# rust-control/oxide_control

Hardware: NVIDIA B200
Metric: env-steps/sec (higher is better)
Workload: dtype f32

## Files before the change

oxide_control_b200/csrc/ox_jit.cpp:

```cpp
#include <cuda_runtime_api.h>
#include <sys/stat.h>
#include <unistd.h>

#include <atomic>
#include <cerrno>
#include <cinttypes>
#include <cstdio>
#include <cstdlib>
#include <fstream>
#include <map>
#include <memory>
#include <mutex>
#include <sstream>
#include <string>
#include <vector>

#include "ox_specsrc.h"

#define OX_INCBIN(sym, file)                                                                                       \
  __asm__(".section .rodata\n.hidden " #sym "\n.global " #sym "\n.balign 16\n" #sym ":\n.incbin \"" file "\"\n"   \
          ".hidden " #sym "_end\n.global " #sym "_end\n" #sym "_end:\n.byte 0\n.previous\n");                      \
  extern "C" const char sym[];                                                                                     \
  extern "C" const char sym##_end[];
OX_INCBIN(ox_embed_spec_cuh, "ox_spec.cuh")
OX_INCBIN(ox_embed_stages_cuh, "ox_stages.cuh")
OX_INCBIN(ox_embed_blob_h, "ox_blob.h")
OX_INCBIN(ox_embed_abi_h, "../../include/ox_b200.h")

namespace ox {
namespace {

const char* kFlags = "-std=c++17 -O3 -lineinfo -gencode arch=compute_100a,code=sm_100a --expt-relaxed-constexpr -cubin";

struct Embedded { const char* rel; const char* begin; const char* end; };
const Embedded* embedded(int* n) {
  static const Embedded e[] = {
      {"src/csrc/ox_spec.cuh", ox_embed_spec_cuh, ox_embed_spec_cuh_end},
      {"src/csrc/ox_stages.cuh", ox_embed_stages_cuh, ox_embed_stages_cuh_end},
      {"src/csrc/ox_blob.h", ox_embed_blob_h, ox_embed_blob_h_end},
      {"include/ox_b200.h", ox_embed_abi_h, ox_embed_abi_h_end},
  };
  *n = 4;
  return e;
}

uint64_t fnv(uint64_t h, const void* p, size_t n) {
  const unsigned char* c = static_cast<const unsigned char*>(p);
  for (size_t i = 0; i < n; i++) { h ^= c[i]; h *= 1099511628211ull; }
  return h;
}
uint64_t abi_hash() {
  static const uint64_t h = [] {
    uint64_t x = 1469598103934665603ull;
    int n;
    const Embedded* e = embedded(&n);
    for (int i = 0; i < n; i++) x = fnv(x, e[i].begin, (size_t)(e[i].end - e[i].begin));
    x = fnv(x, kFlags, strlen(kFlags));
    return x;
  }();
  return h;
}

bool mkdirs(const std::string& path) {
  std::string cur;
  for (size_t i = 0; i <= path.size(); i++) {
    if (i == path.size() || path[i] == '/') {
      if (!cur.empty() && mkdir(cur.c_str(), 0755) != 0 && errno != EEXIST) return false;
    }
    if (i < path.size()) cur += path[i];
  }
  return true;
}
bool write_file(const std::string& path, const char* data, size_t n) {
  std::ofstream f(path, std::ios::binary);
  if (!f) return false;
  f.write(data, (std::streamsize)n);
  return (bool)f;
}
bool read_file(const std::string& path, std::vector<char>* out) {
  std::ifstream f(path, std::ios::binary);
  if (!f) return false;
  out->assign(std::istreambuf_iterator<char>(f), std::istreambuf_iterator<char>());
  return !out->empty();
}
std::string cache_dir() {
  if (const char* d = getenv("OX_B200_CACHE_DIR")) if (*d) return d;
  if (const char* d = getenv("XDG_CACHE_HOME")) if (*d) return std::string(d) + "/ox_b200";
  if (const char* d = getenv("HOME")) if (*d) return std::string(d) + "/.cache/ox_b200";
  return "/tmp/ox_b200_cache";
}
std::string find_nvcc() {
  auto ok = [](const std::string& p) { return !p.empty() && access(p.c_str(), X_OK) == 0; };
  if (const char* p = getenv("OX_B200_NVCC")) if (ok(p)) return p;
  for (const char* v : {"CUDA_HOME", "CUDA_PATH"})
    if (const char* d = getenv(v)) { std::string p = std::string(d) + "/bin/nvcc"; if (ok(p)) return p; }
  if (ok("/usr/local/cuda/bin/nvcc")) return "/usr/local/cuda/bin/nvcc";
  if (const char* path = getenv("PATH")) {
    std::stringstream ss(path);
    std::string dir;
    while (std::getline(ss, dir, ':')) { std::string p = dir + "/nvcc"; if (ok(p)) return p; }
  }
  return "";
}
std::string shq(const std::string& s) {
  std::string r = "'";
  for (char c : s) { if (c == '\'') r += "'\\''"; else r += c; }
  return r + "'";
}
std::string tail(const std::string& path, size_t n) {
  std::vector<char> d;
  if (!read_file(path, &d)) return "";
  return std::string(d.size() > n ? d.end() - (long)n : d.begin(), d.end());
}

bool compile_unit(const ox_model_tables& t, bool f64, const std::string& cubin, std::string* why) {
  const std::string nvcc = find_nvcc();
  if (nvcc.empty()) { *why = "nvcc not found (set OX_B200_NVCC or CUDA_HOME)"; return false; }
  static std::atomic<int> counter{0};
  const std::string dir = cache_dir();
  char tmpname[64];
  snprintf(tmpname, sizeof tmpname, "/build_%ld_%d", (long)getpid(), counter++);
  const std::string work = dir + tmpname;
  if (!mkdirs(work + "/src/csrc") || !mkdirs(work + "/include")) { *why = "cannot create " + work; return false; }
  int n;
  const Embedded* e = embedded(&n);
  for (int i = 0; i < n; i++)
    if (!write_file(work + "/" + e[i].rel, e[i].begin, (size_t)(e[i].end - e[i].begin))) { *why = "cannot write " + work + "/" + e[i].rel; return false; }
  const std::string src = spec_source_jit(t, f64);
  if (!write_file(work + "/src/csrc/spec.cu", src.data(), src.size())) { *why = "cannot write spec.cu"; return false; }
  const std::string cmd = shq(nvcc) + " " + kFlags + " -I" + shq(work + "/src/csrc") + " -o " + shq(work + "/spec.cubin") + " " +
                          shq(work + "/src/csrc/spec.cu") + " > " + shq(work + "/nvcc.log") + " 2>&1";
  const int rc = system(cmd.c_str());
  std::vector<char> probe;
  if (rc != 0 || !read_file(work + "/spec.cubin", &probe)) {
    *why = "nvcc failed (rc " + std::to_string(rc) + "): " + tail(work + "/nvcc.log", 600) + " [sources kept in " + work + "]";
    return false;
  }
  if (rename((work + "/spec.cubin").c_str(), cubin.c_str()) != 0) { *why = "cannot move the cubin into " + cubin; return false; }
  const std::string rm = "rm -rf " + shq(work);
  if (system(rm.c_str()) != 0) {  }
  return true;
}

struct JitEntry {
  SpecEntry spec;
  std::string name;
  cudaLibrary_t lib[2] = {nullptr, nullptr};
  std::string cubin[2];
};
std::mutex g_mu;
std::map<uint64_t, std::unique_ptr<JitEntry>>& table() {
  static std::map<uint64_t, std::unique_ptr<JitEntry>> t;
  return t;
}

}

bool jit_enabled() {
  const char* v = getenv("OX_B200_JIT");
  return !(v && v[0] == '0');
}

const SpecEntry* jit_spec(const ox_model_tables& t, bool f64, bool allow_compile, bool load, std::string* why, std::string* cubin_path) {
  std::string dummy;
  if (!why) why = &dummy;
  if (!jit_enabled()) { *why = "run-time specialisation disabled (OX_B200_JIT=0)"; return nullptr; }
  const uint64_t hash = model_hash(t);
  std::lock_guard<std::mutex> lock(g_mu);
  auto& slot = table()[hash];
  if (!slot) {
    slot.reset(new JitEntry);
    char nm[64];
    snprintf(nm, sizeof nm, "jit_%016" PRIx64, hash);
    slot->name = nm;
    slot->spec.hash = hash;
    slot->spec.name = slot->name.c_str();
  }
  JitEntry& je = *slot;
  const int p = f64 ? 1 : 0;
  void** kern = f64 ? je.spec.jit_f64 : je.spec.jit_f32;
  if (je.cubin[p].empty()) {
    const std::string dir = cache_dir();
    if (!mkdirs(dir)) { *why = "cannot create the cache directory " + dir; return nullptr; }
    char fn[128];
    snprintf(fn, sizeof fn, "/ox_%016" PRIx64 "_%s_%016" PRIx64 ".cubin", hash, f64 ? "f64" : "f32", abi_hash());
    const std::string path = dir + fn;
    if (access(path.c_str(), R_OK) != 0) {
      if (!allow_compile) { *why = "no cached cubin for this model (" + path + ")"; return nullptr; }
      if (!compile_unit(t, f64, path, why)) return nullptr;
    }
    je.cubin[p] = path;
  }
  if (cubin_path) *cubin_path = je.cubin[p];
  if (!load) return &je.spec;
  if (!kern[0]) {
    std::vector<char> image;
    if (!read_file(je.cubin[p], &image)) { *why = "cannot read " + je.cubin[p]; return nullptr; }
    cudaLibrary_t lib = nullptr;
    cudaError_t err = cudaLibraryLoadData(&lib, image.data(), nullptr, nullptr, 0, nullptr, nullptr, 0);
    if (err != cudaSuccess) { *why = std::string("cudaLibraryLoadData: ") + cudaGetErrorString(err); cudaGetLastError(); return nullptr; }
    cudaKernel_t k0 = nullptr, k1 = nullptr, k2 = nullptr;
    err = cudaLibraryGetKernel(&k0, lib, "ox_jit_step");
    if (err != cudaSuccess) { *why = std::string("cudaLibraryGetKernel(ox_jit_step): ") + cudaGetErrorString(err); cudaGetLastError(); cudaLibraryUnload(lib); return nullptr; }
    if (spec_wants_split(t)) {
      if (cudaLibraryGetKernel(&k1, lib, "ox_jit_pre") != cudaSuccess || cudaLibraryGetKernel(&k2, lib, "ox_jit_post") != cudaSuccess) {
        cudaGetLastError(); k1 = k2 = nullptr;
      }
    }
    je.lib[p] = lib;
// ... 8 lines not shown
```

oxide_control_b200/csrc/ox_stages.cuh:

```cuda
#pragma once
#include <cmath>

#include "ox_blob.h"

namespace ox {

OX_HD float ox_sqrt(float x) { return sqrtf(x); }
OX_HD double ox_sqrt(double x) { return sqrt(x); }
OX_HD float ox_rsqrt(float x) {
#if defined(__CUDA_ARCH__)
  return rsqrtf(x);
#else
  return 1.0f / sqrtf(x);
#endif
}
OX_HD double ox_rsqrt(double x) {
#if defined(__CUDA_ARCH__)
  return rsqrt(x);
#else
  return 1.0 / sqrt(x);
#endif
}
OX_HD float ox_abs(float x) { return fabsf(x); }
OX_HD double ox_abs(double x) { return fabs(x); }
// ... 1696 lines not shown
          if (!body) continue;
          const int last_ = m.body_dofadr(body) + m.body_dofnum(body) - 1;
          OX_MLOOP
          for (int d_ = 0, dof = last_; d_ < m.dof_depth(last_); d_++, dof = m.dof_parentid(dof)) {
            T cd[6];
            ld<6>(cd, b.cdof, 6 * dof);
            OX_MLOOP
            for (int k = 0; k < 3; k++) at(b.efc_J, (q0 + k) * nv + dof) += sign * (G[3 * k] * cd[0] + G[3 * k + 1] * cd[1] + G[3 * k + 2] * cd[2]);
          }
        }
        const T rdiag = m.body_invweight0(2 * b1 + 1) + m.body_invweight0(2 * b2 + 1);
        OX_MLOOP
        for (int k = 0; k < 3; k++) eq_row_finish(i, q0 + k, res[k], rdiag);
      }
    } else {
      const int j1 = m.eq_obj1id(i), j2 = m.eq_obj2id(i);
      const int d1 = m.jnt_dofadr(j1), q1 = m.jnt_qposadr(j1);
      const int r = nefc++;
      OX_MLOOP
      for (int k = 0; k < nv; k++) at(b.efc_J, r * nv + k) = 0;
      T c[5];
      OX_LDM(5, c, eq_data, 11 * i);
      T pos = at(b.qpos, q1) - m.qpos0(q1), diag = m.dof_invweight0(d1);
      at(b.efc_J, r * nv + d1) = 1;
      if (j2 >= 0) {
        const int d2 = m.jnt_dofadr(j2), q2 = m.jnt_qposadr(j2);
        const T dq = at(b.qpos, q2) - m.qpos0(q2);
        pos -= c[0] + dq * (c[1] + dq * (c[2] + dq * (c[3] + dq * c[4])));
        at(b.efc_J, r * nv + d2) = -(c[1] + dq * (2 * c[2] + dq * (3 * c[3] + dq * 4 * c[4])));
        diag += m.dof_invweight0(d2);
      } else {
        pos -= c[0];
      }
      eq_row_finish(i, r, pos, diag);
    }
  }
  OX_HD void friction_row(int i, int& nefc) const {
    const T fl = m.dof_frictionloss(i);
    if (!(fl > 0)) return;
    const int nv = m.h().nv, r = nefc++;
    OX_MLOOP
    for (int k = 0; k < nv; k++) at(b.efc_J, r * nv + k) = 0;
    at(b.efc_J, r * nv + i) = 1;
    T aref, sr[2], si[5];
    OX_LDM(2, sr, dof_solref_fri, 2 * i);
    OX_LDM(5, si, dof_solimp_fri, 5 * i);
    const T R = row_params(sr, si, (T)0, (T)0, m.dof_invweight0(i), at(b.qvel, i), &aref);
    at(b.efc_pos, r) = 0; at(b.efc_margin, r) = 0; at(b.efc_D, r) = 1 / R; at(b.efc_aref, r) = aref; at(b.efc_floss, r) = fl;
  }
  OX_HD T ball_angle_axis(int j, T* axis) const {
    T q[4];
    ld<4>(q, b.qpos, m.jnt_qposadr(j));
    normalize4(q);
    const T sn = ox_sqrt(q[1] * q[1] + q[2] * q[2] + q[3] * q[3]);
    T ang = 2 * ox_atan2(sn, q[0]);
    if (ang > (T)3.14159265358979323846) ang -= (T)(2 * 3.14159265358979323846);
    const T inv = sn > (T)OX_MINVAL ? 1 / sn : (T)0;
    const T sg = ang < 0 ? (T)-1 : (T)1;
    axis[0] = sg * q[1] * inv; axis[1] = sg * q[2] * inv; axis[2] = sg * q[3] * inv;
    return ox_abs(ang);
  }
  OX_HD int limit_count(int j) const {
    if (!m.jnt_limited(j)) return 0;
    const int jt = m.jnt_type(j);
    if (jt == OX_JNT_BALL) {
      T axis[3];
      return ox_max(m.jnt_range(2 * j), m.jnt_range(2 * j + 1)) - ball_angle_axis(j, axis) < m.jnt_margin(j) ? 1 : 0;
    }
    if (jt != OX_JNT_SLIDE && jt != OX_JNT_HINGE) return 0;
    const T value = at(b.qpos, m.jnt_qposadr(j)), margin = m.jnt_margin(j);
    return (value - m.jnt_range(2 * j) < margin ? 1 : 0) + (m.jnt_range(2 * j + 1) - value < margin ? 1 : 0);
  }
  OX_HD void limit_rows(int j, int& nefc) const {
    const int nv = m.h().nv;
    {
      {
          if (!m.jnt_limited(j)) return;
          const int jt = m.jnt_type(j);
          if (jt == OX_JNT_BALL) {
            T axis[3];
            const T margin = m.jnt_margin(j), dist = ox_max(m.jnt_range(2 * j), m.jnt_range(2 * j + 1)) - ball_angle_axis(j, axis);
            if (!(dist < margin)) return;
            const int da = m.jnt_dofadr(j), r = nefc++;
            OX_MLOOP
            for (int i = 0; i < nv; i++) at(b.efc_J, r * nv + i) = 0;
            T vel = 0;
            OX_MLOOP
            for (int k = 0; k < 3; k++) { at(b.efc_J, r * nv + da + k) = -axis[k]; vel -= axis[k] * at(b.qvel, da + k); }
            T aref, sr[2], si[5];
            OX_LDM(2, sr, jnt_solref, 2 * j);
            OX_LDM(5, si, jnt_solimp, 5 * j);
            const T R = row_params(sr, si, dist, margin, m.dof_invweight0(da), vel, &aref);
            at(b.efc_pos, r) = dist; at(b.efc_margin, r) = margin; at(b.efc_D, r) = 1 / R; at(b.efc_aref, r) = aref;
            return;
          }
          if (jt != OX_JNT_SLIDE && jt != OX_JNT_HINGE) return;
          const int da = m.jnt_dofadr(j);
          const T value = at(b.qpos, m.jnt_qposadr(j)), margin = m.jnt_margin(j);
          OX_MLOOP
          for (int side = -1; side <= 1; side += 2) {
            const T dist = side * (m.jnt_range(2 * j + (side + 1) / 2) - value);
            if (dist < margin) {
              const int r = nefc++;
              OX_MLOOP
              for (int i = 0; i < nv; i++) at(b.efc_J, r * nv + i) = 0;
              at(b.efc_J, r * nv + da) = (T)(-side);
              const T vel = (T)(-side) * at(b.qvel, da);
              T aref;
              T sr[2], si[5];
              OX_LDM(2, sr, jnt_solref, 2 * j);
              OX_LDM(5, si, jnt_solimp, 5 * j);
              const T R = row_params(sr, si, dist, margin, m.dof_invweight0(da), vel, &aref);
              at(b.efc_pos, r) = dist; at(b.efc_margin, r) = margin; at(b.efc_D, r) = 1 / R; at(b.efc_aref, r) = aref;
            }
          }
      }
    }
  }

  OX_HD int tendon_limit_count(int i) const {
    if (!m.tendon_limited(i)) return 0;
    const T value = at(b.ten_length, i), margin = m.tendon_margin(i);
    return (value - m.tendon_range(2 * i) < margin ? 1 : 0) + (m.tendon_range(2 * i + 1) - value < margin ? 1 : 0);
  }
  OX_HD void tendon_limit_rows(int i, int& nefc) const {
    const int nv = m.h().nv;
    if (!m.tendon_limited(i)) return;
    const T value = at(b.ten_length, i), margin = m.tendon_margin(i);
    OX_MLOOP
    for (int side = -1; side <= 1; side += 2) {
      const T dist = side * (m.tendon_range(2 * i + (side + 1) / 2) - value);
      if (dist < margin) {
        const int r = nefc++;
        OX_MLOOP
        for (int k = 0; k < nv; k++) at(b.efc_J, r * nv + k) = 0;
        T vel = 0;
        OX_MLOOP
        for (int k = 0; k < nv; k++) {
          const T c = (T)(-side) * at(b.ten_J, i * nv + k);
          at(b.efc_J, r * nv + k) = c;
          vel += c * at(b.qvel, k);
        }
        T aref, sr[2], si[5];
        OX_LDM(2, sr, tendon_solref_lim, 2 * i);
        OX_LDM(5, si, tendon_solimp_lim, 5 * i);
        const T R = row_params(sr, si, dist, margin, m.tendon_invweight0(i), vel, &aref);
        at(b.efc_pos, r) = dist; at(b.efc_margin, r) = margin; at(b.efc_D, r) = 1 / R; at(b.efc_aref, r) = aref;
      }
    }
  }

  struct LsPt { T alpha, cost, d0, d1, s0; };

  OX_HD LsPt ls_eval(T a, int nefc, T qg0, T qg1, T qg2) const {
    const int ne_ = ati(b.ne, 0), nfe_ = ne_ + ati(b.nf, 0);
    LsPt p;
    p.alpha = a;
    p.cost = a * a * qg2 + a * qg1 + qg0;
    p.d0 = 2 * a * qg2 + qg1;
    p.d1 = 2 * qg2;
    p.s0 = ox_abs(2 * a * qg2) + ox_abs(qg1);
    OX_ROWLOOP
    const bool ell_ = m.h().cone == OX_CONE_ELLIPTIC;
    if (ell_)
      for_each_contact([&](int, int pp, int ea, int dim) {
        if (dim == 1) return;
        T x[6], D[6], jvv[6], f[6], Hc[36], ck;
#pragma unroll
        for (int j = 0; j < 6; j++) { if (j >= dim) break; jvv[j] = at(b.s_Jv, ea + j); x[j] = at(b.s_Jaref, ea + j) + a * jvv[j]; D[j] = at(b.efc_D, ea + j); }
        elliptic_cost(pp, dim, D, x, &ck, f, Hc);
        p.cost += ck;
#pragma unroll
        for (int j = 0; j < 6; j++) {
          if (j >= dim) break;
          p.d0 -= f[j] * jvv[j];
          p.s0 += ox_abs(f[j] * jvv[j]);
#pragma unroll
          for (int l = 0; l < 6; l++) { if (l >= dim) break; p.d1 += jvv[j] * Hc[j * dim + l] * jvv[l]; }
        }
      });
    for (int r = 0; r < nefc; r++) {
      if (ell_ && r >= nfe_ && at(b.efc_floss, r) < 0) continue;
      const T ja = at(b.s_Jaref, r), jv = at(b.s_Jv, r);
      const T x = ja + a * jv;
      if (r >= ne_ && r < nfe_) {
        const T fl = at(b.efc_floss, r), D = at(b.efc_D, r);
        if (ox_abs(x) * D >= fl) {
          const T sg = x > 0 ? (T)1 : (T)-1;
          p.cost += fl * (sg * x - (T)0.5 * fl / D);
          p.d0 += sg * fl * jv;
          p.s0 += ox_abs(fl * jv);
          continue;
        }
      }
      if (x < 0 || r < nfe_) {
        const T Dx = at(b.efc_D, r) * x, Dj = at(b.efc_D, r) * jv;
        p.cost += (T)0.5 * Dx * x;
        p.d0 += Dx * jv;
        p.d1 += Dj * jv;
        p.s0 += ox_abs(Dx * jv);
      }
    }
    if (p.d1 < (T)OX_MINVAL) p.d1 = (T)OX_MINVAL;
    return p;
  }

  OX_HD T update_constraint(int nv, int nefc, T* gauss_out) const {
    const int ne_ = ati(b.ne, 0), nfe_ = ne_ + ati(b.nf, 0);
    T c = 0;
    OX_NVLOOP
    for (int i = 0; i < nv; i++) at(b.qfrc_constraint, i) = 0;
    const bool ell_ = m.h().cone == OX_CONE_ELLIPTIC;
    if (ell_)
      for_each_contact([&](int, int pp, int ea, int dim) {
        if (dim == 1) return;
        T x[6], D[6], f[6], ck;
#pragma unroll
        for (int j = 0; j < 6; j++) { if (j >= dim) break; x[j] = at(b.s_Jaref, ea + j); D[j] = at(b.efc_D, ea + j); }
        elliptic_cost(pp, dim, D, x, &ck, f, (T*)nullptr);
        c += ck;
#pragma unroll
        for (int j = 0; j < 6; j++) {
          if (j >= dim) break;
          at(b.efc_force, ea + j) = f[j];
          if (f[j] != 0) {
            OX_NVLOOP
            for (int i = 0; i < nv; i++) at(b.qfrc_constraint, i) += at(b.efc_J, (ea + j) * nv + i) * f[j];
          }
        }
      });
    OX_ROWLOOP
    for (int r = 0; r < nefc; r++) {
      if (ell_ && r >= nfe_ && at(b.efc_floss, r) < 0) continue;
      const T ja = at(b.s_Jaref, r);
      T f = 0;
      if (r >= ne_ && r < nfe_ && ox_abs(ja) * at(b.efc_D, r) >= at(b.efc_floss, r)) {
        const T fl = at(b.efc_floss, r), sg = ja > 0 ? (T)1 : (T)-1;
        f = -sg * fl;
        c += fl * (sg * ja - (T)0.5 * fl / at(b.efc_D, r));
        OX_NVLOOP
        for (int i = 0; i < nv; i++) at(b.qfrc_constraint, i) += at(b.efc_J, r * nv + i) * f;
      } else if (ja < 0 || r < nfe_) {
        const T D = at(b.efc_D, r);
        f = -D * ja;
        c += (T)0.5 * D * ja * ja;
        OX_NVLOOP
        for (int i = 0; i < nv; i++) at(b.qfrc_constraint, i) += at(b.efc_J, r * nv + i) * f;
      }
      at(b.efc_force, r) = f;
    }
    T g = 0;
    OX_NVLOOP
    for (int i = 0; i < nv; i++) g += (T)0.5 * (at(b.s_Ma, i) - at(b.qfrc_smooth, i)) * (at(b.qacc, i) - at(b.qacc_smooth, i));
    *gauss_out = g;
    return c + g;
  }

  OX_HD T update_gradient(int nv, int nefc, bool newton) const {
    T gn = 0;
    OX_NVLOOP
    for (int i = 0; i < nv; i++) {
      const T g = at(b.s_Ma, i) - at(b.qfrc_smooth, i) - at(b.qfrc_constraint, i);
      at(b.s_grad, i) = g;
      gn += g * g;
    }
    if (!newton) {
      OX_NVLOOP
      for (int i = 0; i < nv; i++) at(b.s_Mgrad, i) = at(b.s_grad, i);
      solve_ld(b.s_Mgrad);
      return ox_sqrt(gn);
    }
    T* H = b.s_H;
    const int ne_ = ati(b.ne, 0), nfe_ = ne_ + ati(b.nf, 0);
    OX_NVLOOP
    for (int i = 0; i < nv; i++) {
      OX_NVLOOP
      for (int j = 0; j <= i; j++) at(H, i * nv + j) = 0;
      int adr = m.dof_Madr(i);
      OX_NVLOOP
      for (int d_ = 0, j = i; d_ < m.dof_depth(i); d_++, j = m.dof_parentid(j)) at(H, i * nv + j) = at(b.qM, adr++);
    }
    OX_ROWLOOP
    for (int r = 0; r < nefc; r++) {
      if (r >= ne_ && r < nfe_) { if (ox_abs(at(b.s_Jaref, r)) * at(b.efc_D, r) >= at(b.efc_floss, r)) continue; }
      else if (m.h().cone == OX_CONE_ELLIPTIC && r >= nfe_ && at(b.efc_floss, r) < 0) continue;
      else if (!(at(b.s_Jaref, r) < 0 || r < ne_)) continue;
      const T D = at(b.efc_D, r);
      if constexpr (UNROLL_NV) {
        constexpr int NV = M::Hdr::nv;
        T Jr[NV > 0 ? NV : 1];
#pragma unroll
        for (int i = 0; i < NV; i++) Jr[i] = at(b.efc_J, r * NV + i);
#pragma unroll
        for (int i = 0; i < NV; i++) {
          const T s = D * Jr[i];
#pragma unroll
          for (int j = 0; j <= i; j++) at(H, i * NV + j) += s * Jr[j];
        }
      } else {
        for (int i = 0; i < nv; i++) {
          const T ji = at(b.efc_J, r * nv + i);
          if (ji == 0) continue;
          const T s = D * ji;
          for (int j = 0; j <= i; j++) at(H, i * nv + j) += s * at(b.efc_J, r * nv + j);
        }
      }
    }
    if (m.h().cone == OX_CONE_ELLIPTIC)
      for_each_contact([&](int, int pp, int ea, int dim) {
        if (dim == 1) return;
        T x[6], D[6], Hc[36], ck;
#pragma unroll
        for (int j = 0; j < 6; j++) { if (j >= dim) break; x[j] = at(b.s_Jaref, ea + j); D[j] = at(b.efc_D, ea + j); }
        if (elliptic_cost(pp, dim, D, x, &ck, (T*)nullptr, Hc) == 0) return;
        for (int a = 0; a < dim; a++)
          for (int c2 = 0; c2 < dim; c2++) {
            const T hh = Hc[a * dim + c2];
            if (hh == 0) continue;
            for (int i = 0; i < nv; i++) {
              const T sa = hh * at(b.efc_J, (ea + a) * nv + i);
              if (sa == 0) continue;
              for (int j = 0; j <= i; j++) at(H, i * nv + j) += sa * at(b.efc_J, (ea + c2) * nv + j);
            }
          }
      });
    OX_NVLOOP
    for (int j = 0; j < nv; j++) {
      T s = at(H, j * nv + j);
      OX_NVLOOP
      for (int k = 0; k < j; k++) { const T l = at(H, j * nv + k); s -= l * l; }
      const T inv = ox_rsqrt(ox_max(s, (T)OX_MINVAL));
      at(H, j * nv + j) = inv;
      OX_NVLOOP
      for (int i = j + 1; i < nv; i++) {
        T v = at(H, i * nv + j);
        OX_NVLOOP
        for (int k = 0; k < j; k++) v -= at(H, i * nv + k) * at(H, j * nv + k);
        at(H, i * nv + j) = v * inv;
      }
    }
    OX_NVLOOP
    for (int i = 0; i < nv; i++) {
      T v = at(b.s_grad, i);
      OX_NVLOOP
      for (int k = 0; k < i; k++) v -= at(H, i * nv + k) * at(b.s_Mgrad, k);
      at(b.s_Mgrad, i) = v * at(H, i * nv + i);
    }
    OX_NVLOOP
    for (int i = nv - 1; i >= 0; i--) {
      T v = at(b.s_Mgrad, i);
      OX_NVLOOP
      for (int k = i + 1; k < nv; k++) v -= at(H, k * nv + i) * at(b.s_Mgrad, k);
      at(b.s_Mgrad, i) = v * at(H, i * nv + i);
    }
    return ox_sqrt(gn);
  }

  OX_HD T cost_at(const T* qacc, int nv, int nefc) const {
    const int ne_ = ati(b.ne, 0), nfe_ = ne_ + ati(b.nf, 0);
    const bool ell_ = m.h().cone == OX_CONE_ELLIPTIC;
    mul_m(b.s_Mv, qacc);
    T c = 0;
    OX_NVLOOP
    for (int i = 0; i < nv; i++) c += (T)0.5 * (at(b.s_Mv, i) - at(b.qfrc_smooth, i)) * (at(qacc, i) - at(b.qacc_smooth, i));
    OX_ROWLOOP
    for (int r = 0; r < nefc; r++) {
      T v = -at(b.efc_aref, r);
      OX_NVLOOP
      for (int i = 0; i < nv; i++) v += at(b.efc_J, r * nv + i) * at(qacc, i);
      if (ell_) at(b.s_Jv, r) = v;
      if (ell_ && r >= nfe_ && at(b.efc_floss, r) < 0) continue;
      if (r >= ne_ && r < nfe_ && ox_abs(v) * at(b.efc_D, r) >= at(b.efc_floss, r)) c += at(b.efc_floss, r) * (ox_abs(v) - (T)0.5 * at(b.efc_floss, r) / at(b.efc_D, r));
      else if (v < 0 || r < nfe_) c += (T)0.5 * at(b.efc_D, r) * v * v;
    }
    if (ell_)
      for_each_contact([&](int, int pp, int ea, int dim) {
        if (dim == 1) return;
        T x[6], D[6], ck;
#pragma unroll
        for (int j = 0; j < 6; j++) { if (j >= dim) break; x[j] = at(b.s_Jv, ea + j); D[j] = at(b.efc_D, ea + j); }
        elliptic_cost(pp, dim, D, x, &ck, (T*)nullptr, (T*)nullptr);
        c += ck;
      });
    return c;
  }

  OX_HD T row_dot(int r, const T* v, int nv) const {
    T s = 0;
    OX_NVLOOP
    for (int i = 0; i < nv; i++) s += at(b.efc_J, r * nv + i) * at(v, i);
    return s;
  }
  OX_HD void dual_to_primal(int nv, int nefc) const {
    OX_NVLOOP
    for (int i = 0; i < nv; i++) at(b.qfrc_constraint, i) = 0;
    OX_ROWLOOP
    for (int r = 0; r < nefc; r++) {
      const T f = at(b.efc_force, r);
      if (f == 0) continue;
      OX_NVLOOP
      for (int i = 0; i < nv; i++) at(b.qfrc_constraint, i) += at(b.efc_J, r * nv + i) * f;
    }
    OX_NVLOOP
    for (int i = 0; i < nv; i++) at(b.s_Ma, i) = at(b.qfrc_constraint, i);
    solve_ld(b.s_Ma);
    OX_NVLOOP
    for (int i = 0; i < nv; i++) at(b.s_Ma, i) += at(b.qacc_smooth, i);
  }
  OX_HD void dual_pgs(int nv, int nefc) const {
    const auto& h = m.h();
    const int ne_ = ati(b.ne, 0), nfe_ = ne_ + ati(b.nf, 0);
    const T scale = 1 / ((T)h.meaninertia * (T)(nv > 1 ? nv : 1));
    bool warm = false;
    if (!dis(OX_DSBL_WARMSTART)) {
      OX_ROWLOOP
      for (int r = 0; r < nefc; r++) {
        const T jar = row_dot(r, b.qacc_warmstart, nv) - at(b.efc_aref, r);
        T f = (jar < 0 || r < nfe_) ? -at(b.efc_D, r) * jar : (T)0;
        if (r >= ne_ && r < nfe_) f = ox_clip(f, -at(b.efc_floss, r), at(b.efc_floss, r));
        at(b.efc_force, r) = f;
      }
      dual_to_primal(nv, nefc);
      T cost = 0;
      OX_ROWLOOP
      for (int r = 0; r < nefc; r++) {
        const T f = at(b.efc_force, r), jw = row_dot(r, b.s_Ma, nv), js = row_dot(r, b.qacc_smooth, nv);
        cost += (T)0.5 * f * (jw - js + f / at(b.efc_D, r)) + f * (js - at(b.efc_aref, r));
      }
      warm = cost < 0;
    }
    if (!warm) {
      OX_ROWLOOP
      for (int r = 0; r < nefc; r++) at(b.efc_force, r) = 0;
      OX_NVLOOP
      for (int i = 0; i < nv; i++) at(b.s_Ma, i) = at(b.qacc_smooth, i);
    }
    int iter = 0;
    const int maxiter = h.iterations;
    const T tol = (T)h.tolerance;
#pragma unroll 1
    while (iter < maxiter) {
      T improvement = 0;
#pragma unroll 1
      for (int r = 0; r < nefc; r++) {
        OX_NVLOOP
        for (int i = 0; i < nv; i++) at(b.s_Mv, i) = at(b.efc_J, r * nv + i);
        solve_ld(b.s_Mv);
        const T R = 1 / at(b.efc_D, r), ARrr = row_dot(r, b.s_Mv, nv) + R;
        const T old = at(b.efc_force, r);
        const T res = row_dot(r, b.s_Ma, nv) - at(b.efc_aref, r) + R * old;
        T f = old - res / ARrr;
        if (r >= ne_ && r < nfe_) f = ox_clip(f, -at(b.efc_floss, r), at(b.efc_floss, r));
        else if (r >= ne_ && f < 0) f = 0;
        const T delta = f - old;
        if (delta != 0) {
          at(b.efc_force, r) = f;
          OX_NVLOOP
          for (int i = 0; i < nv; i++) at(b.s_Ma, i) += delta * at(b.s_Mv, i);
          improvement -= (T)0.5 * delta * delta * ARrr + delta * res;
        }
      }
      iter++;
      if (improvement * scale < tol) break;
    }
    ati(b.solver_niter, 0) = iter;
  }
  OX_HD T noslip_pair(int ra, int rb, int nv) const {
    OX_NVLOOP
    for (int i = 0; i < nv; i++) at(b.s_Mv, i) = at(b.efc_J, ra * nv + i) - at(b.efc_J, rb * nv + i);
    solve_ld(b.s_Mv);
    const T K = row_dot(ra, b.s_Mv, nv) - row_dot(rb, b.s_Mv, nv);
    if (K < (T)OX_MINVAL) return 0;
    const T fa = at(b.efc_force, ra), fb = at(b.efc_force, rb), mid = (T)0.5 * (fa + fb), yold = (T)0.5 * (fa - fb);
    const T dres = (row_dot(ra, b.s_Ma, nv) - at(b.efc_aref, ra)) - (row_dot(rb, b.s_Ma, nv) - at(b.efc_aref, rb));
    T y = yold - dres / K;
    y = ox_max(-mid, ox_min(mid, y));
    const T delta = y - yold;
    if (delta == 0) return 0;
    at(b.efc_force, ra) = mid + y; at(b.efc_force, rb) = mid - y;
    OX_NVLOOP
    for (int i = 0; i < nv; i++) at(b.s_Ma, i) += delta * at(b.s_Mv, i);
    return -((T)0.5 * delta * delta * K + delta * dres);
  }
  OX_HD T noslip_contact(int c, int p, int nv) const {
    const int ea = ati(b.con_efcadr, c), dim = m.pair_dim(p);
    T imp = 0;
    if (ea < 0 || dim < 3) return imp;
#pragma unroll 1
    for (int k = 0; k < dim - 1; k++) imp += noslip_pair(ea + 2 * k, ea + 2 * k + 1, nv);
    return imp;
  }
  OX_HD void dual_noslip(int nv, int nefc) const {
    const auto& h = m.h();
    const T scale = 1 / ((T)h.meaninertia * (T)(nv > 1 ? nv : 1));
    dual_to_primal(nv, nefc);
#pragma unroll 1
    const int ne_ = ati(b.ne, 0), nfe_ = ne_ + ati(b.nf, 0);
#pragma unroll 1
    for (int iter = 0; iter < h.noslip_iterations; iter++) {
      T improvement = 0;
#pragma unroll 1
      for (int r = ne_; r < nfe_; r++) {
        OX_NVLOOP
        for (int i = 0; i < nv; i++) at(b.s_Mv, i) = at(b.efc_J, r * nv + i);
        solve_ld(b.s_Mv);
        const T Arr = row_dot(r, b.s_Mv, nv);
        if (Arr < (T)OX_MINVAL) continue;
        const T old = at(b.efc_force, r), res = row_dot(r, b.s_Ma, nv) - at(b.efc_aref, r);
        const T f = ox_clip(old - res / Arr, -at(b.efc_floss, r), at(b.efc_floss, r)), delta = f - old;
        if (delta != 0) {
          at(b.efc_force, r) = f;
          OX_NVLOOP
          for (int i = 0; i < nv; i++) at(b.s_Ma, i) += delta * at(b.s_Mv, i);
          improvement -= (T)0.5 * delta * delta * Arr + delta * res;
        }
      }
      if (STATIC_CON || slots) {
#pragma unroll 1
        for (int p = 0; p < h.npair; p++)
#pragma unroll 1
          for (int k = 0; k < m.pair_maxcon(p); k++) {
            const int c = m.pair_conadr(p) + k;
            if (ati(b.con_active, c)) improvement += noslip_contact(c, p, nv);
          }
      } else {
        const int ncon = ati(b.ncon, 0);
#pragma unroll 1
        for (int c = 0; c < ncon; c++) improvement += noslip_contact(c, ati(b.con_pair, c), nv);
      }
      if (improvement * scale < (T)h.noslip_tolerance) break;
    }
  }
  OX_HD void dual_finish(int nv, int nefc) const {
    dual_to_primal(nv, nefc);
    OX_NVLOOP
    for (int i = 0; i < nv; i++) { const T a = at(b.s_Ma, i); at(b.qacc, i) = a; at(b.qacc_warmstart, i) = a; }
  }

  OX_HDN void fwd_constraint() const {
    const auto& h = m.h();
    const int nv = h.nv, nefc = ati(b.nefc, 0);
    if (nefc == 0) {
      OX_NVLOOP
      for (int i = 0; i < nv; i++) {
        const T a = at(b.qacc_smooth, i);
        at(b.qacc, i) = a; at(b.qacc_warmstart, i) = a; at(b.qfrc_constraint, i) = 0;
      }
      ati(b.solver_niter, 0) = 0;
      return;
    }
    if (h.solver == OX_SOL_PGS) {
      dual_pgs(nv, nefc);
      if (h.noslip_iterations > 0) dual_noslip(nv, nefc);
      dual_finish(nv, nefc);
      return;
    }
    const bool newton = h.solver == OX_SOL_NEWTON;
    bool use_smooth = true;
    if (!dis(OX_DSBL_WARMSTART)) {
      T cand[2];
#pragma unroll 1
      for (int k = 0; k < 2; k++) {
        OX_NVLOOP
        for (int i = 0; i < nv; i++) at(b.qacc, i) = k ? at(b.qacc_smooth, i) : at(b.qacc_warmstart, i);
        cand[k] = cost_at(b.qacc, nv, nefc);
      }
      use_smooth = cand[0] > cand[1];
    }
    OX_NVLOOP
    for (int i = 0; i < nv; i++) at(b.qacc, i) = use_smooth ? at(b.qacc_smooth, i) : at(b.qacc_warmstart, i);
    mul_m(b.s_Ma, b.qacc);
    OX_ROWLOOP
    for (int r = 0; r < nefc; r++) {
      T v = -at(b.efc_aref, r);
      OX_NVLOOP
      for (int i = 0; i < nv; i++) v += at(b.efc_J, r * nv + i) * at(b.qacc, i);
      at(b.s_Jaref, r) = v;
    }
    T gauss = 0, cost = 0, gnorm = 0;
    const T tol = (T)h.tolerance;
    const T mscale = (T)h.meaninertia * (T)(nv > 1 ? nv : 1);
    const T scale = 1 / mscale;
    const int maxiter = h.iterations;
    int iter = 0;
    bool init = true;
#pragma unroll 1
    for (;;) {
      if (!init) {
        if (iter >= maxiter) break;
        T snorm = 0;
        OX_NVLOOP
        for (int i = 0; i < nv; i++) { const T s = at(b.s_search, i); snorm += s * s; }
        snorm = ox_sqrt(snorm);
        if (snorm < (T)OX_MINVAL) break;
        const T gtol = tol * (T)h.ls_tolerance * snorm * mscale;
        mul_m(b.s_Mv, b.s_search);
        OX_ROWLOOP
        for (int r = 0; r < nefc; r++) {
          T v = 0;
          OX_NVLOOP
          for (int i = 0; i < nv; i++) v += at(b.efc_J, r * nv + i) * at(b.s_search, i);
          at(b.s_Jv, r) = v;
        }
        T qg1 = 0, qg2 = 0;
        OX_NVLOOP
        for (int i = 0; i < nv; i++) {
          const T s = at(b.s_search, i);
          qg1 += s * (at(b.s_Ma, i) - at(b.qfrc_smooth, i));
          qg2 += (T)0.5 * s * at(b.s_Mv, i);
        }
        LsPt p0, lo, hi, cur;
        bool have_hi = false, descent = true;
        T a = 0;
#pragma unroll 1
        for (int it = -1; it < h.ls_iterations; it++) {
          if (it >= 0) {
            a = cur.alpha - cur.d0 / cur.d1;
            if (have_hi && !(a > lo.alpha && a < hi.alpha)) a = (T)0.5 * (lo.alpha + hi.alpha);
            if (ox_abs(a - cur.alpha) <= Eps<T>::v() * ox_abs(a)) break;
          }
          cur = ls_eval(a, nefc, gauss, qg1, qg2);
          if (it < 0) {
            p0 = cur; lo = cur; hi = cur;
            if (!(p0.d0 < 0)) { descent = false; break; }
          } else {
            if (ox_abs(cur.d0) < gtol || ox_abs(cur.d0) <= 8 * Eps<T>::v() * cur.s0) break;
            if (cur.d0 < 0) lo = cur; else { hi = cur; have_hi = true; }
          }
        }
        if (!descent) break;
        const T alpha = cur.cost <= p0.cost ? cur.alpha : 0;
        if (alpha == 0) break;
        OX_NVLOOP
        for (int i = 0; i < nv; i++) {
          at(b.qacc, i) += alpha * at(b.s_search, i);
          at(b.s_Ma, i) += alpha * at(b.s_Mv, i);
          if (!newton) { at(b.s_gradold, i) = at(b.s_grad, i); at(b.s_Mgradold, i) = at(b.s_Mgrad, i); }
        }
        OX_ROWLOOP
        for (int r = 0; r < nefc; r++) at(b.s_Jaref, r) += alpha * at(b.s_Jv, r);
      }
      const T oldcost = cost;
      cost = update_constraint(nv, nefc, &gauss);
      gnorm = update_gradient(nv, nefc, newton);
      bool first = init;
      if (init) {
        init = false;
        if (scale * gnorm < tol) break;
      } else {
        iter++;
        const T improvement = scale * (oldcost - cost), gradient = scale * gnorm;
        if (improvement < tol || gradient < tol) break;
        if (oldcost - cost <= OX_FLOOR_MULT * Eps<T>::v() * (ox_abs(oldcost) + ox_abs(cost))) break;
      }
      if (newton || first) {
        OX_NVLOOP
        for (int i = 0; i < nv; i++) at(b.s_search, i) = -at(b.s_Mgrad, i);
      } else {
        T num = 0, den = 0;
        OX_NVLOOP
        for (int i = 0; i < nv; i++) {
          num += at(b.s_grad, i) * (at(b.s_Mgrad, i) - at(b.s_Mgradold, i));
          den += at(b.s_gradold, i) * at(b.s_Mgradold, i);
        }
        T beta = num / ox_max((T)OX_MINVAL, den);
        if (beta < 0) beta = 0;
        OX_NVLOOP
        for (int i = 0; i < nv; i++) at(b.s_search, i) = -at(b.s_Mgrad, i) + beta * at(b.s_search, i);
      }
    }
    ati(b.solver_niter, 0) = iter;
    if (h.noslip_iterations > 0) {
      dual_noslip(nv, nefc);
      dual_finish(nv, nefc);
      return;
    }
    OX_NVLOOP
    for (int i = 0; i < nv; i++) at(b.qacc_warmstart, i) = at(b.qacc, i);
  }

  static OX_HD T ray_quad(T a, T bq, T c, T* xx) {
    const T det = bq * bq - a * c;
    if (det < (T)OX_MINVAL) { xx[0] = -1; xx[1] = -1; return -1; }
    const T sq = ox_sqrt(det);
    xx[0] = (-bq - sq) / a; xx[1] = (-bq + sq) / a;
    if (xx[0] >= 0) return xx[0];
    if (xx[1] >= 0) return xx[1];
    return -1;
  }
  static OX_HD T ray_geom(const T* pos, const T* mat, const T* size, const T* pnt, const T* vec, int type) {
    const T dif[3] = {pnt[0] - pos[0], pnt[1] - pos[1], pnt[2] - pos[2]};
    T lp[3], lv[3];
#pragma unroll
    for (int k = 0; k < 3; k++) {
      lp[k] = mat[k] * dif[0] + mat[3 + k] * dif[1] + mat[6 + k] * dif[2];
      lv[k] = mat[k] * vec[0] + mat[3 + k] * vec[1] + mat[6 + k] * vec[2];
    }
    T xx[2];
    if (type == OX_GEOM_SPHERE) return ray_quad(dot3(lv, lv), dot3(lv, lp), dot3(lp, lp) - size[0] * size[0], xx);
    T x = -1;
    if (type == OX_GEOM_BOX) {
#pragma unroll
      for (int i = 0; i < 3; i++) {
        if (ox_abs(lv[i]) > (T)OX_MINVAL) {
#pragma unroll
          for (int side = -1; side <= 1; side += 2) {
            const T sol = ((T)side * size[i] - lp[i]) / lv[i];
            if (sol >= 0) {
              const int i0 = (i + 1) % 3, i1 = (i + 2) % 3;
              const T p0 = lp[i0] + sol * lv[i0], p1 = lp[i1] + sol * lv[i1];
              if (ox_abs(p0) <= size[i0] && ox_abs(p1) <= size[i1] && (x < 0 || sol < x)) x = sol;
            }
          }
        }
      }
      return x;
    }
    T sol = ray_quad(lv[0] * lv[0] + lv[1] * lv[1], lv[0] * lp[0] + lv[1] * lp[1], lp[0] * lp[0] + lp[1] * lp[1] - size[0] * size[0], xx);
    if (sol >= 0 && ox_abs(lp[2] + sol * lv[2]) <= size[1]) x = sol;
#pragma unroll
    for (int side = -1; side <= 1; side += 2) {
      const T ld_[3] = {lp[0], lp[1], lp[2] - (T)side * size[1]};
      ray_quad(dot3(lv, lv), dot3(lv, ld_), dot3(ld_, ld_) - size[0] * size[0], xx);
#pragma unroll
      for (int i = 0; i < 2; i++) {
        const T z = lp[2] + xx[i] * lv[2];
        if (xx[i] >= 0 && (side > 0 ? z >= size[1] : z <= -size[1]) && (x < 0 || xx[i] < x)) x = xx[i];
      }
    }
    return x;
  }

  OX_HD void obj_frame(int objtype, int id, T* pos, T* mat, int* body) const {
    if (objtype == OX_OBJ_BODY) { ld<3>(pos, b.xipos, 3 * id); ld<9>(mat, b.ximat, 9 * id); *body = id; }
    else if (objtype == OX_OBJ_XBODY) { ld<3>(pos, b.xpos, 3 * id); ld<9>(mat, b.xmat, 9 * id); *body = id; }
    else if (objtype == OX_OBJ_GEOM) { ld<3>(pos, b.geom_xpos, 3 * id); ld<9>(mat, b.geom_xmat, 9 * id); *body = m.geom_bodyid(id); }
    else { ld<3>(pos, b.site_xpos, 3 * id); ld<9>(mat, b.site_xmat, 9 * id); *body = m.site_bodyid(id); }
  }
  OX_HD void body_acc() const {
    const auto& h = m.h();
    OX_MLOOP
    for (int k = 0; k < 3; k++) { at(b.cacc, k) = 0; at(b.cacc, 3 + k) = dis(OX_DSBL_GRAVITY) ? (T)0 : -(T)h.grav(k); }
    OX_MLOOP
    for (int bd = 1; bd < h.nbody; bd++) {
      T a[6];
      ld<6>(a, b.cacc, 6 * m.body_parentid(bd));
      OX_MLOOP
      for (int d_ = 0; d_ < m.body_dofnum(bd); d_++) {
        const int i = m.body_dofadr(bd) + d_;
        T cd[6], cdd[6];
        ld<6>(cd, b.cdof, 6 * i);
        ld<6>(cdd, b.cdof_dot, 6 * i);
        const T v = at(b.qvel, i), qa = at(b.qacc, i);
        OX_MLOOP
        for (int k = 0; k < 6; k++) a[k] += cdd[k] * v + cd[k] * qa;
      }
      st<6>(b.cacc, 6 * bd, a);
    }
  }
  OX_HD void sub_ext_force(int body, const T* point, const T* force, const T* torque, T sign) const {
    if (body == 0) return;
    T sc[3], dif[3], t[3];
    ld<3>(sc, b.subtree_com, 3 * m.body_rootid(body));
    dif[0] = point[0] - sc[0]; dif[1] = point[1] - sc[1]; dif[2] = point[2] - sc[2];
    cross3(t, dif, force);
    OX_MLOOP
    for (int k = 0; k < 3; k++) {
      at(b.cfrc, 6 * body + k) -= sign * (t[k] + (torque ? torque[k] : (T)0));
      at(b.cfrc, 6 * body + 3 + k) -= sign * force[k];
    }
  }
  OX_HD void cfrc_int() const {
    const auto& h = m.h();
    const int nbody = h.nbody;
    OX_MLOOP
    for (int bd = 1; bd < nbody; bd++) {
      T in[10], ca[6], cv[6], ia[6], iv[6], cf[6];
      ld<10>(in, b.cinert, 10 * bd);
      ld<6>(ca, b.cacc, 6 * bd);
      ld<6>(cv, b.cvel, 6 * bd);
      mul_inert_vec(ia, in, ca);
      mul_inert_vec(iv, in, cv);
      cross_force(cf, cv, iv);
      OX_MLOOP
      for (int k = 0; k < 6; k++) ia[k] += cf[k];
      st<6>(b.cfrc, 6 * bd, ia);
    }
    OX_MLOOP
    for (int bd = 1; bd < nbody; bd++) {
      T f[6], xi[3];
      ld<6>(f, b.xfrc_applied, 6 * bd);
      if (f[0] == 0 && f[1] == 0 && f[2] == 0 && f[3] == 0 && f[4] == 0 && f[5] == 0) continue;
      ld<3>(xi, b.xipos, 3 * bd);
      sub_ext_force(bd, xi, f, f + 3, (T)1);
    }
    auto one = [&](int c, int p) {
      const int ea = ati(b.con_efcadr, c);
      if (ea < 0) return;
      const int dim = m.pair_dim(p);
      T lf[6] = {0, 0, 0, 0, 0, 0};
      if (dim == 1) lf[0] = at(b.efc_force, ea);
      else if (h.cone == OX_CONE_ELLIPTIC) {
#pragma unroll
        for (int k = 0; k < 6; k++) { if (k >= dim) break; lf[k] = at(b.efc_force, ea + k); }
      } else {
#pragma unroll
        for (int k = 0; k < 5; k++) {
// ... 505 lines not shown
```

Baseline: 104.4 million.

## Fuse line-search alpha=0 eval into Jv pass, reuse warmstart products, skip final Hessian

```diff
diff --git a/oxide_control_b200/csrc/ox_jit.cpp b/oxide_control_b200/csrc/ox_jit.cpp
--- a/oxide_control_b200/csrc/ox_jit.cpp
+++ b/oxide_control_b200/csrc/ox_jit.cpp
@@ -26,6 +26,7 @@
 OX_INCBIN(ox_embed_stages_cuh, "ox_stages.cuh")
 OX_INCBIN(ox_embed_blob_h, "ox_blob.h")
 OX_INCBIN(ox_embed_abi_h, "../../include/ox_b200.h")
+OX_INCBIN(ox_embed_specsrc_h, "ox_specsrc.h")
 
 namespace ox {
 namespace {
@@ -55,6 +56,7 @@
     int n;
     const Embedded* e = embedded(&n);
     for (int i = 0; i < n; i++) x = fnv(x, e[i].begin, (size_t)(e[i].end - e[i].begin));
+    x = fnv(x, ox_embed_specsrc_h, (size_t)(ox_embed_specsrc_h_end - ox_embed_specsrc_h));
     x = fnv(x, kFlags, strlen(kFlags));
     return x;
   }();
diff --git a/oxide_control_b200/csrc/ox_stages.cuh b/oxide_control_b200/csrc/ox_stages.cuh
--- a/oxide_control_b200/csrc/ox_stages.cuh
+++ b/oxide_control_b200/csrc/ox_stages.cuh
@@ -1872,15 +1872,42 @@
 
   struct LsPt { T alpha, cost, d0, d1, s0; };
 
-  OX_HD LsPt ls_eval(T a, int nefc, T qg0, T qg1, T qg2) const {
-    const int ne_ = ati(b.ne, 0), nfe_ = ne_ + ati(b.nf, 0);
+  static OX_HD LsPt ls_head(T a, T qg0, T qg1, T qg2) {
     LsPt p;
     p.alpha = a;
     p.cost = a * a * qg2 + a * qg1 + qg0;
     p.d0 = 2 * a * qg2 + qg1;
     p.d1 = 2 * qg2;
     p.s0 = ox_abs(2 * a * qg2) + ox_abs(qg1);
-    OX_ROWLOOP
+    return p;
+  }
+  OX_HD void ls_row(LsPt& p, T a, int r, int ne_, int nfe_, T ja, T jv) const {
+    const T x = ja + a * jv;
+    if (r >= ne_ && r < nfe_) {
+      const T fl = at(b.efc_floss, r), D = at(b.efc_D, r);
+      if (ox_abs(x) * D >= fl) {
+        const T sg = x > 0 ? (T)1 : (T)-1;
+        p.cost += fl * (sg * x - (T)0.5 * fl / D);
+        p.d0 += sg * fl * jv;
+        p.s0 += ox_abs(fl * jv);
+        return;
+      }
+    }
+    if (x < 0 || r < nfe_) {
+      const T Dx = at(b.efc_D, r) * x, Dj = at(b.efc_D, r) * jv;
+      p.cost += (T)0.5 * Dx * x;
+      p.d0 += Dx * jv;
+      p.d1 += Dj * jv;
+      p.s0 += ox_abs(Dx * jv);
+    }
+  }
+  static OX_HD void ls_tail(LsPt& p) {
+    if (p.d1 < (T)OX_MINVAL) p.d1 = (T)OX_MINVAL;
+  }
+
+  OX_HD LsPt ls_eval(T a, int nefc, T qg0, T qg1, T qg2) const {
+    const int ne_ = ati(b.ne, 0), nfe_ = ne_ + ati(b.nf, 0);
+    LsPt p = ls_head(a, qg0, qg1, qg2);
     const bool ell_ = m.h().cone == OX_CONE_ELLIPTIC;
     if (ell_)
       for_each_contact([&](int, int pp, int ea, int dim) {
@@ -1899,29 +1926,12 @@
           for (int l = 0; l < 6; l++) { if (l >= dim) break; p.d1 += jvv[j] * Hc[j * dim + l] * jvv[l]; }
         }
       });
+    OX_ROWLOOP
     for (int r = 0; r < nefc; r++) {
       if (ell_ && r >= nfe_ && at(b.efc_floss, r) < 0) continue;
-      const T ja = at(b.s_Jaref, r), jv = at(b.s_Jv, r);
-      const T x = ja + a * jv;
-      if (r >= ne_ && r < nfe_) {
-        const T fl = at(b.efc_floss, r), D = at(b.efc_D, r);
-        if (ox_abs(x) * D >= fl) {
-          const T sg = x > 0 ? (T)1 : (T)-1;
-          p.cost += fl * (sg * x - (T)0.5 * fl / D);
-          p.d0 += sg * fl * jv;
-          p.s0 += ox_abs(fl * jv);
-          continue;
-        }
-      }
-      if (x < 0 || r < nfe_) {
-        const T Dx = at(b.efc_D, r) * x, Dj = at(b.efc_D, r) * jv;
-        p.cost += (T)0.5 * Dx * x;
-        p.d0 += Dx * jv;
-        p.d1 += Dj * jv;
-        p.s0 += ox_abs(Dx * jv);
-      }
-    }
-    if (p.d1 < (T)OX_MINVAL) p.d1 = (T)OX_MINVAL;
+      ls_row(p, a, r, ne_, nfe_, at(b.s_Jaref, r), at(b.s_Jv, r));
+    }
+    ls_tail(p);
     return p;
   }
 
@@ -1976,7 +1986,7 @@
     return c + g;
   }
 
-  OX_HD T update_gradient(int nv, int nefc, bool newton) const {
+  OX_HD T update_gradient(int nv) const {
     T gn = 0;
     OX_NVLOOP
     for (int i = 0; i < nv; i++) {
@@ -1984,11 +1994,15 @@
       at(b.s_grad, i) = g;
       gn += g * g;
     }
+    return ox_sqrt(gn);
+  }
+
+  OX_HD void update_mgrad(int nv, int nefc, bool newton) const {
     if (!newton) {
       OX_NVLOOP
       for (int i = 0; i < nv; i++) at(b.s_Mgrad, i) = at(b.s_grad, i);
       solve_ld(b.s_Mgrad);
-      return ox_sqrt(gn);
+      return;
     }
     T* H = b.s_H;
     const int ne_ = ati(b.ne, 0), nfe_ = ne_ + ati(b.nf, 0);
@@ -2073,7 +2087,6 @@
       for (int k = i + 1; k < nv; k++) v -= at(H, k * nv + i) * at(b.s_Mgrad, k);
       at(b.s_Mgrad, i) = v * at(H, i * nv + i);
     }
-    return ox_sqrt(gn);
   }
 
   OX_HD T cost_at(const T* qacc, int nv, int nefc) const {
@@ -2088,7 +2101,7 @@
       T v = -at(b.efc_aref, r);
       OX_NVLOOP
       for (int i = 0; i < nv; i++) v += at(b.efc_J, r * nv + i) * at(qacc, i);
-      if (ell_) at(b.s_Jv, r) = v;
+      at(b.s_Jv, r) = v;
       if (ell_ && r >= nfe_ && at(b.efc_floss, r) < 0) continue;
       if (r >= ne_ && r < nfe_ && ox_abs(v) * at(b.efc_D, r) >= at(b.efc_floss, r)) c += at(b.efc_floss, r) * (ox_abs(v) - (T)0.5 * at(b.efc_floss, r) / at(b.efc_D, r));
       else if (v < 0 || r < nfe_) c += (T)0.5 * at(b.efc_D, r) * v * v;
@@ -2276,7 +2289,12 @@
       return;
     }
     const bool newton = h.solver == OX_SOL_NEWTON;
-    bool use_smooth = true;
+    const auto keep_start = [&]() {
+      OX_NVLOOP
+      for (int i = 0; i < nv; i++) at(b.s_Ma, i) = at(b.s_Mv, i);
+      OX_ROWLOOP
+      for (int r = 0; r < nefc; r++) at(b.s_Jaref, r) = at(b.s_Jv, r);
+    };
     if (!dis(OX_DSBL_WARMSTART)) {
       T cand[2];
 #pragma unroll 1
@@ -2284,30 +2302,38 @@
         OX_NVLOOP
         for (int i = 0; i < nv; i++) at(b.qacc, i) = k ? at(b.qacc_smooth, i) : at(b.qacc_warmstart, i);
         cand[k] = cost_at(b.qacc, nv, nefc);
-      }
-      use_smooth = cand[0] > cand[1];
-    }
-    OX_NVLOOP
-    for (int i = 0; i < nv; i++) at(b.qacc, i) = use_smooth ? at(b.qacc_smooth, i) : at(b.qacc_warmstart, i);
-    mul_m(b.s_Ma, b.qacc);
-    OX_ROWLOOP
-    for (int r = 0; r < nefc; r++) {
-      T v = -at(b.efc_aref, r);
+        if (k == 0) keep_start();
+      }
+      if (cand[0] > cand[1]) {
+        keep_start();
+      } else {
+        OX_NVLOOP
+        for (int i = 0; i < nv; i++) at(b.qacc, i) = at(b.qacc_warmstart, i);
+      }
+    } else {
       OX_NVLOOP
-      for (int i = 0; i < nv; i++) v += at(b.efc_J, r * nv + i) * at(b.qacc, i);
-      at(b.s_Jaref, r) = v;
+      for (int i = 0; i < nv; i++) at(b.qacc, i) = at(b.qacc_smooth, i);
+      mul_m(b.s_Ma, b.qacc);
+      OX_ROWLOOP
+      for (int r = 0; r < nefc; r++) {
+        T v = -at(b.efc_aref, r);
+        OX_NVLOOP
+        for (int i = 0; i < nv; i++) v += at(b.efc_J, r * nv + i) * at(b.qacc, i);
+        at(b.s_Jaref, r) = v;
+      }
     }
     T gauss = 0, cost = 0, gnorm = 0;
     const T tol = (T)h.tolerance;
     const T mscale = (T)h.meaninertia * (T)(nv > 1 ? nv : 1);
     const T scale = 1 / mscale;
     const int maxiter = h.iterations;
+    const bool ell_ = h.cone == OX_CONE_ELLIPTIC;
+    const int ne_ = ati(b.ne, 0), nfe_ = ne_ + ati(b.nf, 0);
     int iter = 0;
     bool init = true;
 #pragma unroll 1
     for (;;) {
       if (!init) {
-        if (iter >= maxiter) break;
         T snorm = 0;
         OX_NVLOOP
         for (int i = 0; i < nv; i++) { const T s = at(b.s_search, i); snorm += s * s; }
@@ -2315,21 +2341,23 @@
         if (snorm < (T)OX_MINVAL) break;
         const T gtol = tol * (T)h.ls_tolerance * snorm * mscale;
         mul_m(b.s_Mv, b.s_search);
+        T qg1 = 0, qg2 = 0;
+        OX_NVLOOP
+        for (int i = 0; i < nv; i++) {
+          const T s = at(b.s_search, i);
+          qg1 += s * (at(b.s_Ma, i) - at(b.qfrc_smooth, i));
+          qg2 += (T)0.5 * s * at(b.s_Mv, i);
+        }
+        LsPt p0, lo, hi, cur = ls_head((T)0, gauss, qg1, qg2);
         OX_ROWLOOP
         for (int r = 0; r < nefc; r++) {
           T v = 0;
           OX_NVLOOP
           for (int i = 0; i < nv; i++) v += at(b.efc_J, r * nv + i) * at(b.s_search, i);
           at(b.s_Jv, r) = v;
-        }
-        T qg1 = 0, qg2 = 0;
-        OX_NVLOOP
-        for (int i = 0; i < nv; i++) {
-          const T s = at(b.s_search, i);
-          qg1 += s * (at(b.s_Ma, i) - at(b.qfrc_smooth, i));
-          qg2 += (T)0.5 * s * at(b.s_Mv, i);
-        }
-        LsPt p0, lo, hi, cur;
+          if (!ell_) ls_row(cur, (T)0, r, ne_, nfe_, at(b.s_Jaref, r), v);
+        }
+        ls_tail(cur);
         bool have_hi = false, descent = true;
         T a = 0;
 #pragma unroll 1
@@ -2339,7 +2367,7 @@
             if (have_hi && !(a > lo.alpha && a < hi.alpha)) a = (T)0.5 * (lo.alpha + hi.alpha);
             if (ox_abs(a - cur.alpha) <= Eps<T>::v() * ox_abs(a)) break;
           }
-          cur = ls_eval(a, nefc, gauss, qg1, qg2);
+          if (it >= 0 || ell_) cur = ls_eval(a, nefc, gauss, qg1, qg2);
           if (it < 0) {
             p0 = cur; lo = cur; hi = cur;
             if (!(p0.d0 < 0)) { descent = false; break; }
@@ -2362,7 +2390,7 @@
       }
       const T oldcost = cost;
       cost = update_constraint(nv, nefc, &gauss);
-      gnorm = update_gradient(nv, nefc, newton);
+      gnorm = update_gradient(nv);
       bool first = init;
       if (init) {
         init = false;
@@ -2373,6 +2401,8 @@
         if (improvement < tol || gradient < tol) break;
         if (oldcost - cost <= OX_FLOOR_MULT * Eps<T>::v() * (ox_abs(oldcost) + ox_abs(cost))) break;
       }
+      if (iter >= maxiter) break;
+      update_mgrad(nv, nefc, newton);
       if (newton || first) {
         OX_NVLOOP
         for (int i = 0; i < nv; i++) at(b.s_search, i) = -at(b.s_Mgrad, i);
```

Result: faster. 107.0 million (median of 6 runs) (+2.5%).
